# MTG/DeepConvSep

Hardware: NVIDIA H100
Metric: audio_seconds_separated_per_second (higher is better)
Workload: dtype f32

## Files before the change

### deepconvsep_b200/csrc/fft_reg.cuh

```cuda
#pragma once
#include <cuda_runtime.h>
#include "fft.cuh"

namespace dcs {

__device__ __forceinline__ constexpr float cos32(int q) {
  constexpr float t[16] = {1.0f, 0.98078528040323043f, 0.92387953251128674f, 0.83146961230254524f, 0.70710678118654752f,
                           0.55557023301960218f, 0.38268343236508977f, 0.19509032201612825f, 0.0f, -0.19509032201612825f,
                           -0.38268343236508977f, -0.55557023301960218f, -0.70710678118654752f, -0.83146961230254524f,
                           -0.92387953251128674f, -0.98078528040323043f};
  return t[q];
}
__device__ __forceinline__ constexpr float sin32(int q) {
  constexpr float t[16] = {0.0f, 0.19509032201612825f, 0.38268343236508977f, 0.55557023301960218f, 0.70710678118654752f,
                           0.83146961230254524f, 0.92387953251128674f, 0.98078528040323043f, 1.0f, 0.98078528040323043f,
                           0.92387953251128674f, 0.83146961230254524f, 0.70710678118654752f, 0.55557023301960218f,
                           0.38268343236508977f, 0.19509032201612825f};
  return t[q];
}

__host__ __device__ constexpr int brev(int i, int bits) {
  int r = 0;
  for (int k = 0; k < bits; ++k) r |= ((i >> k) & 1) << (bits - 1 - k);
  return r;
}

__device__ __forceinline__ float2 mul_w32(float2 d, int q) {
  if (q == 0) return d;
  if (q == 8) return make_float2(d.y, -d.x);
  if (q == 4) return make_float2(0.70710678118654752f * (d.x + d.y), 0.70710678118654752f * (d.y - d.x));
  if (q == 12) return make_float2(0.70710678118654752f * (d.y - d.x), -0.70710678118654752f * (d.x + d.y));
  const float c = cos32(q), s = sin32(q);
  return make_float2(fmaf(d.x, c, d.y * s), fmaf(d.y, c, -d.x * s));
}

template <int R, int L = R>
__device__ __forceinline__ void fft_dif(float2 (&v)[R]) {
  constexpr int half = L >> 1;
#pragma unroll
  for (int s = 0; s < R; s += L) {
#pragma unroll
    for (int j = 0; j < half; ++j) {
      const float2 a = v[s + j], b = v[s + j + half];
      v[s + j] = cadd(a, b);
      v[s + j + half] = mul_w32(csub(a, b), j * (32 / L));
    }
  }
  if constexpr (L > 2) fft_dif<R, L / 2>(v);
}

template <int T>
struct FftGroup {
  static constexpr int N2 = 32 * T;
  __device__ static __forceinline__ void fill_tw2(float2* tw2, const float2* __restrict__ tw, int tid, int nthreads) {
    for (int i = tid; i < 32 * T; i += nthreads) {
      const int ka = i / T, b = i - ka * T;
      tw2[i] = __ldg(tw + 2 * b * ka);
    }
  }
  static constexpr int PITCH = T + 1;
  static constexpr int SCRATCH = 32 * PITCH;
  static constexpr int Q = 32 / T;
  static constexpr int TBITS = T == 32 ? 5 : 4;

  template <bool TW_SHARED = false>
  __device__ static __forceinline__ void forward(float2 (&v)[32], float2* scr, const float2* __restrict__ tw, int b) {
    fft_dif<32>(v);
#pragma unroll
    for (int ka = 0; ka < 32; ++ka) {
      float2 y = v[brev(ka, 5)];
      if (ka > 0) y = cmul(y, TW_SHARED ? tw[ka * T + b] : __ldg(tw + 2 * b * ka));
      scr[ka * PITCH + b] = y;
    }
    __syncwarp();
    if (T == 32) {
#pragma unroll
      for (int i = 0; i < 32; ++i) v[i] = scr[b * PITCH + i];
      fft_dif<32>(v);
      float2 u[32];
#pragma unroll
      for (int kb = 0; kb < 32; ++kb) u[kb] = v[brev(kb, 5)];
#pragma unroll
      for (int kb = 0; kb < 32; ++kb) v[kb] = u[kb];
    } else {
      float2 u0[16], u1[16];
#pragma unroll
      for (int i = 0; i < 16; ++i) {
        u0[i] = scr[b * PITCH + i];
        u1[i] = scr[(b + 16) * PITCH + i];
      }
      fft_dif<16>(u0);
      fft_dif<16>(u1);
#pragma unroll
      for (int kb = 0; kb < 16; ++kb) {
        v[kb] = u0[brev(kb, 4)];
        v[16 + kb] = u1[brev(kb, 4)];
      }
    }
    __syncwarp();
  }
};

}
```

### deepconvsep_b200/csrc/stft_reg.cu

```cuda
#include "common.cuh"
#include "fft_reg.cuh"
#include "tc.cuh"

namespace dcs {

constexpr int REG_THREADS = 128;
constexpr int ISTFT_THREADS = 256;

template <int T>
__global__ void __launch_bounds__(REG_THREADS)
stft_reg_kernel(const float* __restrict__ audio, int64_t L, int hop, const float* __restrict__ win,
                const float2* __restrict__ tw, float2* __restrict__ X, float* __restrict__ mag,
                float* __restrict__ phase, int64_t ldf, int64_t nframes, float mag_scale, int frames_per_group) {
  using G = FftGroup<T>;
  constexpr int N2 = G::N2, N = 2 * N2, F = N2 + 1, GPC = REG_THREADS / T;
  extern __shared__ __align__(16) float2 scratch[];
  const int tid = threadIdx.x, b = tid % T, gl = tid / T;
  float2* scr = scratch + gl * G::SCRATCH;
  float2* stw = scratch + GPC * G::SCRATCH;
  float2* stw2 = stw + N2;
  float2* swin = stw2 + N2;
  for (int i = tid; i < N2; i += REG_THREADS) stw[i] = __ldg(tw + i);
  G::fill_tw2(stw2, tw, tid, REG_THREADS);
  for (int i = tid; i < N2; i += REG_THREADS) swin[i] = __ldg(reinterpret_cast<const float2*>(win) + i);
  __syncthreads();
  const int64_t g = (int64_t)blockIdx.x * GPC + gl;
  const bool audio_aligned8 = (reinterpret_cast<uintptr_t>(audio) & 7) == 0;
  const int64_t warp_first = ((int64_t)blockIdx.x * GPC + (tid / 32) * (32 / T)) * frames_per_group;
  for (int i = 0; i < frames_per_group; ++i) {
    if (warp_first + i >= nframes) break;
    const int64_t n = g * frames_per_group + i;
    const bool valid = n < nframes;
    const int64_t base = n * hop - N / 2;
    float2 v[32];
    if (valid && base >= 0 && base + N <= L && audio_aligned8) {
      const float2* __restrict__ ap = reinterpret_cast<const float2*>(audio + base);
#pragma unroll
      for (int a = 0; a < 32; ++a) {
        const int idx = a * T + b;
        const float2 w = swin[idx], x = __ldg(ap + idx);
        v[a] = make_float2(x.x * w.x, x.y * w.y);
      }
    } else {
#pragma unroll
      for (int a = 0; a < 32; ++a) {
        const int idx = a * T + b;
        const int64_t s = base + 2 * idx;
        const float2 w = swin[idx];
        const float x0 = (valid && s >= 0 && s < L) ? __ldg(audio + s) : 0.f;
        const float x1 = (valid && s + 1 >= 0 && s + 1 < L) ? __ldg(audio + s + 1) : 0.f;
        v[a] = make_float2(x0 * w.x, x1 * w.y);
      }
    }
    G::template forward<true>(v, scr, stw2, b);
#pragma unroll
    for (int q = 0; q < G::Q; ++q)
#pragma unroll
      for (int kb = 0; kb < T; ++kb) scr[(b + T * q) + 32 * kb] = v[q * T + kb];
    __syncwarp();
    if (valid) {
      const int64_t row = n * ldf;
#pragma unroll 4
      for (int m = 0; m < N2 / T; ++m) {
        const int k = b + T * m;
        const float2 xk = real_post_shared<N2>(scr, stw, k);
        if (X) X[row + k] = xk;
        if (mag) mag[row + k] = mag_scale * sqrtf(xk.x * xk.x + xk.y * xk.y);
        if (phase) phase[row + k] = atan2f(xk.y, xk.x);
      }
      if (b == 0) {
        const float2 z0 = scr[0];
        const float vv = z0.x - z0.y;
        if (X) X[row + N2] = make_float2(vv, 0.f);
        if (mag) mag[row + N2] = mag_scale * fabsf(vv);
        if (phase) phase[row + N2] = atan2f(0.f, vv);
      }
      if (b < ldf - F) {
        if (X) X[row + F + b] = make_float2(0.f, 0.f);
        if (mag) mag[row + F + b] = 0.f;
        if (phase) phase[row + F + b] = 0.f;
      }
    }
    __syncwarp();
  }
}

constexpr int ISTFT_RING = 2;
constexpr size_t SM90_SMEM_OPTIN = 232448;
template <int T>
__host__ __device__ constexpr int istft_rowp() { return (32 * T + 1 + 7) / 8 * 8; }
template <int T>
__host__ __device__ constexpr size_t istft_smem_bytes(int qpc, bool masked) {
  constexpr int GPC = ISTFT_THREADS / T, ROWP = istft_rowp<T>();
  return ((size_t)GPC * FftGroup<T>::SCRATCH + 3 * (size_t)(32 * T) + (size_t)qpc * ISTFT_RING * ROWP) * sizeof(float2) +
         (masked ? (size_t)GPC * ISTFT_RING * ROWP * sizeof(float) : 0) +
         ((size_t)qpc * 2 * ISTFT_RING + (masked ? (size_t)GPC * ISTFT_RING : 0)) * sizeof(uint64_t);
}

template <int T, int HS, bool MASKED>
__device__ __forceinline__ void
istft_reg_body(const float2* __restrict__ S, int64_t nframes, int64_t ldf, int64_t src_stride,
               const float* __restrict__ wsyn, const float* __restrict__ w2, const float2* __restrict__ tw,
               float* __restrict__ out, int64_t Lout, int64_t out_stride, int hops_per_group, int64_t num_hops,
               int64_t groups_per_src, int64_t total_quads, const float* __restrict__ Mk, int64_t m_stride, int nsrc,
               int nx, int qw, int qpc) {
  using G = FftGroup<T>;
  constexpr int N2 = G::N2, N = 2 * N2, hop = 64 * HS, R = N / hop, C0 = (N / 2) / hop, GPC = ISTFT_THREADS / T;
  constexpr int ROWP = istft_rowp<T>();
  constexpr uint32_t XBYTES = (N2 + 2) / 2 * 16;
  constexpr uint32_t MBYTES = (N2 + 4) / 4 * 16;
  extern __shared__ __align__(16) float2 scratch[];
  const int tid = threadIdx.x, b = tid % T, gl = tid / T;
  float2* scr = scratch + gl * G::SCRATCH;
  const int qi = gl / qw, mem = gl - qi * qw;
  const bool in_quad = qi < qpc;
  int64_t gq = (int64_t)blockIdx.x * qpc + (in_quad ? qi : 0);
  bool active = in_quad && gq < total_quads;
  if (gq >= total_quads) gq = total_quads - 1;
  int msrc = 0;
  if constexpr (MASKED) {
    const int nchunk = (nsrc + qw - 1) / qw;
    msrc = (int)(gq % nchunk) * qw + mem;
    gq /= nchunk;
    if (msrc >= nsrc) { active = false; msrc = nsrc - 1; }
  }
  const int src = (int)(gq / groups_per_src);
  const int64_t h0 = (gq % groups_per_src) * hops_per_group;
  const float inv_n2 = 1.0f / (float)N2;
  float2 acc[32];
#pragma unroll
  for (int i = 0; i < 32; ++i) acc[i] = make_float2(0.f, 0.f);
  float* o = out + (int64_t)(MASKED ? msrc * nx + src : src) * out_stride;
  float2 cinv[G::Q * HS];
#pragma unroll
  for (int q = 0; q < G::Q; ++q)
#pragma unroll
    for (int kb = 0; kb < HS; ++kb) {
      const int e = 2 * ((b + T * q) + 32 * kb);
      float c0 = 0.f, c1 = 0.f;
#pragma unroll
      for (int r = 0; r < R; ++r) {
        const float2 ww = __ldg(reinterpret_cast<const float2*>(w2 + e + r * hop));
        c0 += ww.x;
        c1 += ww.y;
      }
      cinv[q * HS + kb] = make_float2(c0 == 0.f ? 1.f : 1.f / c0, c1 == 0.f ? 1.f : 1.f / c1);
    }

  float2* stw = scratch + GPC * G::SCRATCH;
  float2* stw2 = stw + N2;
  float2* swsyn = stw2 + N2;
  float2* xring = swsyn + N2 + (in_quad ? qi : 0) * ISTFT_RING * ROWP;
  float* mring = reinterpret_cast<float*>(swsyn + N2 + qpc * ISTFT_RING * ROWP) + gl * ISTFT_RING * ROWP;
  uint64_t* bars = reinterpret_cast<uint64_t*>(reinterpret_cast<float*>(swsyn + N2 + qpc * ISTFT_RING * ROWP) +
                                               (MASKED ? GPC * ISTFT_RING * ROWP : 0));
  uint64_t* xfull = bars + (in_quad ? qi : 0) * 2 * ISTFT_RING;
  uint64_t* xempty = xfull + ISTFT_RING;
  uint64_t* mfull = bars + qpc * 2 * ISTFT_RING + gl * ISTFT_RING;
  for (int i = tid; i < N2; i += ISTFT_THREADS) stw[i] = __ldg(tw + i);
  G::fill_tw2(stw2, tw, tid, ISTFT_THREADS);
  for (int i = tid; i < N2; i += ISTFT_THREADS) swsyn[i] = __ldg(reinterpret_cast<const float2*>(wsyn) + i);
  if (tid < qpc * ISTFT_RING) {
    tc::mbar_init(bars + (tid / ISTFT_RING) * 2 * ISTFT_RING + tid % ISTFT_RING, 1);
    tc::mbar_init(bars + (tid / ISTFT_RING) * 2 * ISTFT_RING + ISTFT_RING + tid % ISTFT_RING, (uint32_t)qw);
  }
  if (MASKED && tid < GPC * ISTFT_RING) tc::mbar_init(bars + qpc * 2 * ISTFT_RING + tid, 1);
  tc::fence_barrier_init();
  __syncthreads();
  const bool xlane = in_quad && mem == 0 && b == 0;
  const bool glane = in_quad && b == 0;
  const int64_t n_first = h0 + C0 - R + 1, n_last = h0 + hops_per_group - 1 + C0;
  auto fetch_x = [&](int64_t nn) {
    const int k = (int)(nn - n_first), st = k % ISTFT_RING;
    if (k >= ISTFT_RING)
      tc::mbar_wait_relaxed(xempty + st, (uint32_t)((k / ISTFT_RING - 1) & 1));
    if (nn >= 0 && nn < nframes) {
      tc::mbar_arrive_expect_tx(xfull + st, XBYTES);
      tc::bulk_copy_g2s(xring + st * ROWP, S + (int64_t)src * src_stride + nn * ldf, XBYTES, xfull + st);
    } else {
      tc::mbar_arrive(xfull + st);
    }
  };
  auto fetch_m = [&](int64_t nn) {
    const int st = (int)(nn - n_first) % ISTFT_RING;
    if (nn >= 0 && nn < nframes) {
      tc::mbar_arrive_expect_tx(mfull + st, MBYTES);
      tc::bulk_copy_g2s(mring + st * ROWP, Mk + (int64_t)msrc * m_stride + nn * ldf, MBYTES, mfull + st);
    } else {
      tc::mbar_arrive(mfull + st);
    }
  };
  if (xlane) fetch_x(n_first);
  if (MASKED && glane) fetch_m(n_first);
  for (int64_t n = n_first; n <= n_last; ++n) {
    const bool fvalid = in_quad && n >= 0 && n < nframes;
    const int k = (int)(n - n_first), st = k % ISTFT_RING;
    const uint32_t par = (uint32_t)((k / ISTFT_RING) & 1);
    if (n < n_last) {
      if (xlane) fetch_x(n + 1);
      if (MASKED && glane) fetch_m(n + 1);
    }
    const float2* srow = xring + st * ROWP;
    const float* smrow = mring + st * ROWP;
    if (in_quad) {
      tc::mbar_wait(xfull + st, par);
      if constexpr (MASKED) tc::mbar_wait(mfull + st, par);
    }
    float2 v[32];
#pragma unroll
    for (int a = 0; a < 32; ++a) {
      const int idx = a * T + b;
      float2 xk = make_float2(0.f, 0.f), xn = xk;
      if (fvalid) {
        xk = srow[idx];
        xn = srow[N2 - idx];
        if constexpr (MASKED) {
          const float mk = smrow[idx], mn = smrow[N2 - idx];
          xk = make_float2(__fmul_rn(mk, xk.x), __fmul_rn(mk, xk.y));
          xn = make_float2(__fmul_rn(mn, xn.x), __fmul_rn(mn, xn.y));
        }
      }
      if (idx == 0) { xk.y = 0.f; xn.y = 0.f; }
      v[a] = real_pre_conj(xk, xn, stw[idx]);
    }
    __syncwarp();
    if (glane) tc::mbar_arrive(xempty + st);
    G::template forward<true>(v, scr, stw2, b);
#pragma unroll
    for (int q = 0; q < G::Q; ++q)
#pragma unroll
      for (int kb = 0; kb < T; ++kb) {
        const int np = (b + T * q) + 32 * kb;
        const float2 w = swsyn[np];
        const float2 r = v[q * T + kb];
        acc[q * T + kb].x = fmaf(w.x, r.x * inv_n2, acc[q * T + kb].x);
        acc[q * T + kb].y = fmaf(w.y, -r.y * inv_n2, acc[q * T + kb].y);
      }
    const int64_t h = n - C0;
    if (active && h >= h0 && h < num_hops) {
      const bool interior = (n - (R - 1) >= 0) && (n < nframes);
#pragma unroll
      for (int q = 0; q < G::Q; ++q)
#pragma unroll
        for (int kb = 0; kb < HS; ++kb) {
          const int e = 2 * ((b + T * q) + 32 * kb);
          float2 ic = cinv[q * HS + kb];
          if (!interior) {
            float c0 = 0.f, c1 = 0.f;
#pragma unroll
            for (int r = 0; r < R; ++r) {
              const int64_t nf = n - r;
              if (nf >= 0 && nf < nframes) {
                const float2 ww = __ldg(reinterpret_cast<const float2*>(w2 + e + r * hop));
                c0 += ww.x;
                c1 += ww.y;
              }
            }
            ic = make_float2(c0 == 0.f ? 1.f : 1.f / c0, c1 == 0.f ? 1.f : 1.f / c1);
          }
          const int64_t oi = h * hop + e;
          const float2 a2 = acc[q * T + kb];
          if (oi + 1 < Lout) {
            *reinterpret_cast<float2*>(o + oi) = make_float2(a2.x * ic.x, a2.y * ic.y);
          } else if (oi < Lout) {
            o[oi] = a2.x * ic.x;
          }
        }
    }
#pragma unroll
    for (int q = 0; q < G::Q; ++q) {
#pragma unroll
      for (int kb = 0; kb < T - HS; ++kb) acc[q * T + kb] = acc[q * T + kb + HS];
#pragma unroll
      for (int kb = T - HS; kb < T; ++kb) acc[q * T + kb] = make_float2(0.f, 0.f);
    }
  }
}

template <int T, int HS>
__global__ void __launch_bounds__(ISTFT_THREADS, 1)
istft_reg_kernel(const float2* __restrict__ S, int64_t nframes, int64_t ldf, int64_t src_stride,
                 const float* __restrict__ wsyn, const float* __restrict__ w2, const float2* __restrict__ tw,
                 float* __restrict__ out, int64_t Lout, int64_t out_stride, int hops_per_group, int64_t num_hops,
                 int64_t groups_per_src, int64_t total_groups) {
  istft_reg_body<T, HS, false>(S, nframes, ldf, src_stride, wsyn, w2, tw, out, Lout, out_stride, hops_per_group, num_hops,
                               groups_per_src, total_groups, nullptr, 0, 1, 1, 1, ISTFT_THREADS / T);
}

template <int T, int HS>
__global__ void __launch_bounds__(ISTFT_THREADS, 1)
istft_masked_reg_kernel(const float2* __restrict__ X, int64_t nframes, int64_t ldf, int64_t x_plane,
                        const float* __restrict__ Mk, int64_t m_stride, int nsrc, int nx, const float* __restrict__ wsyn,
                        const float* __restrict__ w2, const float2* __restrict__ tw, float* __restrict__ out, int64_t Lout,
                        int64_t out_stride, int hops_per_group, int64_t num_hops, int64_t groups_per_plane,
                        int64_t total_quads, int qw, int qpc) {
  istft_reg_body<T, HS, true>(X, nframes, ldf, x_plane, wsyn, w2, tw, out, Lout, out_stride, hops_per_group, num_hops,
                              groups_per_plane, total_quads, Mk, m_stride, nsrc, nx, qw, qpc);
}

int launch_stft_reg(dcs_stft* p, const float* d_audio, int64_t L, float2* d_X, float* d_mag, float* d_phase,
                    float mag_scale, int64_t ldf, int64_t nframes, cudaStream_t st) {
  const int fpg = 4;
  const float ms = mag_scale / sqrtf((float)p->N);
  if (p->N == 2048) {
    using G = FftGroup<32>;
    const int gpc = REG_THREADS / 32;
    const size_t smem = (gpc * G::SCRATCH + 3 * G::N2) * sizeof(float2);
    DCS_TRY(ensure_smem_attr(stft_reg_kernel<32>, (int)smem));
    const unsigned grid = (unsigned)ceil_div64(nframes, (int64_t)gpc * fpg);
    stft_reg_kernel<32><<<grid, REG_THREADS, smem, st>>>(
        d_audio, L, p->hop, p->d_win, p->d_tw, d_X, d_mag, d_phase, ldf, nframes, ms, fpg);
  } else {
    using G = FftGroup<16>;
    const int gpc = REG_THREADS / 16;
    const size_t smem = (gpc * G::SCRATCH + 3 * G::N2) * sizeof(float2);
    DCS_TRY(ensure_smem_attr(stft_reg_kernel<16>, (int)smem));
    const unsigned grid = (unsigned)ceil_div64(nframes, (int64_t)gpc * fpg);
    stft_reg_kernel<16><<<grid, REG_THREADS, smem, st>>>(
        d_audio, L, p->hop, p->d_win, p->d_tw, d_X, d_mag, d_phase, ldf, nframes, ms, fpg);
  }
  DCS_CHECK_LAUNCH();
  p->ctx->launches++;
  return DCS_OK;
}

bool istft_reg_supported(const dcs_stft* p, const float* d_out, int64_t out_stride) {
  return (p->N == 1024 || p->N == 2048) && (p->hop == 512 || p->hop == 256) && ((uintptr_t)d_out % 8 == 0) &&
         out_stride % 2 == 0;
}

template <int T, int HS>
static int launch_istft_reg_t(dcs_stft* p, const float2* d_S, int nsrc, int64_t nframes, int64_t ldf, int64_t src_stride,
                              float* d_out, int64_t Lout, int64_t out_stride, cudaStream_t st, const float* d_M = nullptr,
                              int64_t m_stride = 0, int nx = 1) {
  constexpr int GPC = ISTFT_THREADS / T;
  const int hop = 64 * HS;
  const int64_t num_hops = ceil_div64(Lout, hop);
  const int64_t target_groups = (int64_t)p->ctx->num_sms * (ISTFT_THREADS / 32) * (32 / T);
  const int nplanes = nsrc * nx;
  int64_t hpg = ceil_div64((int64_t)nplanes * num_hops, target_groups);
  if (hpg < 12) hpg = 12;
  if (hpg > 64) hpg = 64;
  const int64_t groups_per_src = ceil_div64(num_hops, hpg);
  if (d_M) {
    const int qw = nsrc < GPC ? nsrc : GPC;
    int qpc = GPC / qw;
    while (qpc > 1 && istft_smem_bytes<T>(qpc, true) > SM90_SMEM_OPTIN) --qpc;
    const int64_t quads = groups_per_src * nx * ((nsrc + qw - 1) / qw);
    const unsigned grid = (unsigned)ceil_div64(quads, qpc);
    const size_t smem = istft_smem_bytes<T>(qpc, true);
    DCS_TRY(ensure_smem_attr(istft_masked_reg_kernel<T, HS>, (int)smem));
    istft_masked_reg_kernel<T, HS><<<grid, ISTFT_THREADS, smem, st>>>(
        d_S, nframes, ldf, src_stride, d_M, m_stride, nsrc, nx, p->d_wsyn, p->d_w2, p->d_tw, d_out, Lout, out_stride,
        (int)hpg, num_hops, groups_per_src, quads, qw, qpc);
  } else {
    const int64_t total = groups_per_src * nplanes;
    const unsigned grid = (unsigned)ceil_div64(total, GPC);
    const size_t smem = istft_smem_bytes<T>(GPC, false);
    DCS_TRY(ensure_smem_attr(istft_reg_kernel<T, HS>, (int)smem));
    istft_reg_kernel<T, HS><<<grid, ISTFT_THREADS, smem, st>>>(
        d_S, nframes, ldf, src_stride, p->d_wsyn, p->d_w2, p->d_tw, d_out, Lout, out_stride, (int)hpg, num_hops,
        groups_per_src, total);
  }
  DCS_CHECK_LAUNCH();
  p->ctx->launches++;
  return DCS_OK;
}

int launch_istft_reg(dcs_stft* p, const float2* d_S, int nsrc, int64_t nframes, int64_t ldf, int64_t src_stride,
                     float* d_out, int64_t Lout, int64_t out_stride, cudaStream_t st, const float* d_M, int64_t m_stride,
                     int nx) {
#define DCS_ISTFT_REG_CASE(NN, HOP) \
  if (p->N == NN && p->hop == HOP)  \
    return launch_istft_reg_t<NN / 64, HOP / 64>(p, d_S, nsrc, nframes, ldf, src_stride, d_out, Lout, out_stride, st, d_M, m_stride, nx);
  DCS_ISTFT_REG_CASE(2048, 512)
  DCS_ISTFT_REG_CASE(2048, 256)
  DCS_ISTFT_REG_CASE(1024, 512)
  DCS_ISTFT_REG_CASE(1024, 256)
#undef DCS_ISTFT_REG_CASE
  DCS_REQUIRE(false, "istft_reg: unsupported frame size / hop");
}

}
```

Measured before the change: 162,600.

## Restructure ISTFT overlap-add accumulators and halve FFT scratch for masked kernel

The overlap-add accumulator becomes a per-hop ring of P×HV registers, so the per-frame shift loop over all 32 accumulators goes away. Window normalization and the 1/N scale are folded into the shared synthesis window, and the per-thread inverse-coefficient registers are replaced with a shared-memory table. The masked kernel moves to 384 threads with a half-size FFT transpose scratch, done in two passes via forward_split, to fit more warps per block. Per-warp frame offsets and clamp ranges are precomputed into shared memory to simplify the frame loop. This adds complexity and extra syncwarps, and increases register pressure at the higher thread count.

```diff
diff --git a/deepconvsep_b200/csrc/fft_reg.cuh b/deepconvsep_b200/csrc/fft_reg.cuh
--- a/deepconvsep_b200/csrc/fft_reg.cuh
+++ b/deepconvsep_b200/csrc/fft_reg.cuh
@@ -99,6 +99,59 @@
     }
     __syncwarp();
   }
+
+  static constexpr int HALF_SCRATCH = 16 * PITCH;
+  __device__ static __forceinline__ void forward_split(float2 (&v)[32], float2* scr, const float2* tw, int b) {
+    fft_dif<32>(v);
+    auto y = [&](int ka) { return ka > 0 ? cmul(v[brev(ka, 5)], tw[ka * T + b]) : v[0]; };
+    if (T == 32) {
+      const bool hi = (b & 16) != 0;
+      float2 later[16];
+#pragma unroll
+      for (int a = 0; a < 16; ++a) {
+        const float2 lo = y(a), up = y(a + 16);
+        scr[a * PITCH + b] = hi ? up : lo;
+        later[a] = hi ? lo : up;
+      }
+      const float2* row = scr + (b & 15) * PITCH;
+      __syncwarp();
+#pragma unroll
+      for (int i = 0; i < 16; ++i) v[i] = row[(hi ? 16 : 0) + i];
+      __syncwarp();
+#pragma unroll
+      for (int a = 0; a < 16; ++a) scr[a * PITCH + b] = later[a];
+      __syncwarp();
+#pragma unroll
+      for (int i = 0; i < 16; ++i) v[16 + i] = row[(hi ? 0 : 16) + i];
+      fft_dif<32>(v);
+      float2 u[32];
+#pragma unroll
+      for (int kb = 0; kb < 32; ++kb) u[kb] = v[brev(kb, 5)];
+#pragma unroll
+      for (int kb = 0; kb < 32; ++kb) v[kb] = u[kb];
+    } else {
+      float2 u0[16], u1[16];
+#pragma unroll
+      for (int a = 0; a < 16; ++a) scr[a * PITCH + b] = y(a);
+      __syncwarp();
+#pragma unroll
+      for (int i = 0; i < 16; ++i) u0[i] = scr[b * PITCH + i];
+      __syncwarp();
+#pragma unroll
+      for (int a = 0; a < 16; ++a) scr[a * PITCH + b] = y(16 + a);
+      __syncwarp();
+#pragma unroll
+      for (int i = 0; i < 16; ++i) u1[i] = scr[b * PITCH + i];
+      fft_dif<16>(u0);
+      fft_dif<16>(u1);
+#pragma unroll
+      for (int kb = 0; kb < 16; ++kb) {
+        v[kb] = u0[brev(kb, 4)];
+        v[16 + kb] = u1[brev(kb, 4)];
+      }
+    }
+    __syncwarp();
+  }
 };
 
 }
diff --git a/deepconvsep_b200/csrc/stft_reg.cu b/deepconvsep_b200/csrc/stft_reg.cu
--- a/deepconvsep_b200/csrc/stft_reg.cu
+++ b/deepconvsep_b200/csrc/stft_reg.cu
@@ -6,6 +6,8 @@
 
 constexpr int REG_THREADS = 128;
 constexpr int ISTFT_THREADS = 256;
+constexpr int ISTFT_MASKED_THREADS = 384;
+__host__ __device__ constexpr int istft_threads(bool masked) { return masked ? ISTFT_MASKED_THREADS : ISTFT_THREADS; }
 
 template <int T>
 __global__ void __launch_bounds__(REG_THREADS)
@@ -89,12 +91,20 @@
 constexpr size_t SM90_SMEM_OPTIN = 232448;
 template <int T>
 __host__ __device__ constexpr int istft_rowp() { return (32 * T + 1 + 7) / 8 * 8; }
-template <int T>
+template <int T, int HS>
 __host__ __device__ constexpr size_t istft_smem_bytes(int qpc, bool masked) {
-  constexpr int GPC = ISTFT_THREADS / T, ROWP = istft_rowp<T>();
-  return ((size_t)GPC * FftGroup<T>::SCRATCH + 3 * (size_t)(32 * T) + (size_t)qpc * ISTFT_RING * ROWP) * sizeof(float2) +
-         (masked ? (size_t)GPC * ISTFT_RING * ROWP * sizeof(float) : 0) +
-         ((size_t)qpc * 2 * ISTFT_RING + (masked ? (size_t)GPC * ISTFT_RING : 0)) * sizeof(uint64_t);
+  const int gpc = istft_threads(masked) / T, rowp = istft_rowp<T>();
+  const int scr = masked ? FftGroup<T>::HALF_SCRATCH : FftGroup<T>::SCRATCH;
+  return ((size_t)gpc * scr + 3 * (size_t)(32 * T) + 32 * HS + (size_t)qpc * ISTFT_RING * rowp) * sizeof(float2) +
+         (masked ? (size_t)gpc * ISTFT_RING * rowp * sizeof(float) : 0) +
+         ((size_t)qpc * 2 * ISTFT_RING + (masked ? (size_t)gpc * ISTFT_RING : 0) + 6 * (size_t)gpc) * sizeof(uint64_t);
+}
+
+__device__ __forceinline__ float2 real_pre_conj_x2(float2 xk, float2 xn, float2 twk) {
+  const float2 e = make_float2(xk.x + xn.x, xk.y - xn.y);
+  const float2 d = make_float2(xk.x - xn.x, xk.y + xn.y);
+  const float2 o = cmul(d, make_float2(twk.x, -twk.y));
+  return make_float2(e.x - o.y, -(e.y + o.x));
 }
 
 template <int T, int HS, bool MASKED>
@@ -105,13 +115,17 @@
                int64_t groups_per_src, int64_t total_quads, const float* __restrict__ Mk, int64_t m_stride, int nsrc,
                int nx, int qw, int qpc) {
   using G = FftGroup<T>;
-  constexpr int N2 = G::N2, N = 2 * N2, hop = 64 * HS, R = N / hop, C0 = (N / 2) / hop, GPC = ISTFT_THREADS / T;
+  constexpr int N2 = G::N2, N = 2 * N2, hop = 64 * HS, R = N / hop, C0 = (N / 2) / hop;
+  constexpr int THREADS = istft_threads(MASKED), GPC = THREADS / T;
+  constexpr int SCR = MASKED ? G::HALF_SCRATCH : G::SCRATCH;
+  constexpr int P = R - 1;
+  constexpr int HV = G::Q * HS;
   constexpr int ROWP = istft_rowp<T>();
   constexpr uint32_t XBYTES = (N2 + 2) / 2 * 16;
   constexpr uint32_t MBYTES = (N2 + 4) / 4 * 16;
   extern __shared__ __align__(16) float2 scratch[];
   const int tid = threadIdx.x, b = tid % T, gl = tid / T;
-  float2* scr = scratch + gl * G::SCRATCH;
+  float2* scr = scratch + gl * SCR;
   const int qi = gl / qw, mem = gl - qi * qw;
   const bool in_quad = qi < qpc;
   int64_t gq = (int64_t)blockIdx.x * qpc + (in_quad ? qi : 0);
@@ -126,40 +140,45 @@
   }
   const int src = (int)(gq / groups_per_src);
   const int64_t h0 = (gq % groups_per_src) * hops_per_group;
-  const float inv_n2 = 1.0f / (float)N2;
-  float2 acc[32];
-#pragma unroll
-  for (int i = 0; i < 32; ++i) acc[i] = make_float2(0.f, 0.f);
+  float2 acc[P][HV];
+#pragma unroll
+  for (int p = 0; p < P; ++p)
+#pragma unroll
+    for (int i = 0; i < HV; ++i) acc[p][i] = make_float2(0.f, 0.f);
   float* o = out + (int64_t)(MASKED ? msrc * nx + src : src) * out_stride;
-  float2 cinv[G::Q * HS];
-#pragma unroll
-  for (int q = 0; q < G::Q; ++q)
-#pragma unroll
-    for (int kb = 0; kb < HS; ++kb) {
-      const int e = 2 * ((b + T * q) + 32 * kb);
-      float c0 = 0.f, c1 = 0.f;
-#pragma unroll
-      for (int r = 0; r < R; ++r) {
-        const float2 ww = __ldg(reinterpret_cast<const float2*>(w2 + e + r * hop));
-        c0 += ww.x;
-        c1 += ww.y;
-      }
-      cinv[q * HS + kb] = make_float2(c0 == 0.f ? 1.f : 1.f / c0, c1 == 0.f ? 1.f : 1.f / c1);
-    }
-
-  float2* stw = scratch + GPC * G::SCRATCH;
+
+  float2* stw = scratch + GPC * SCR;
   float2* stw2 = stw + N2;
   float2* swsyn = stw2 + N2;
-  float2* xring = swsyn + N2 + (in_quad ? qi : 0) * ISTFT_RING * ROWP;
-  float* mring = reinterpret_cast<float*>(swsyn + N2 + qpc * ISTFT_RING * ROWP) + gl * ISTFT_RING * ROWP;
-  uint64_t* bars = reinterpret_cast<uint64_t*>(reinterpret_cast<float*>(swsyn + N2 + qpc * ISTFT_RING * ROWP) +
+  float2* scinv = swsyn + N2;
+  float2* xring = scinv + 32 * HS + (in_quad ? qi : 0) * ISTFT_RING * ROWP;
+  float* mring = reinterpret_cast<float*>(scinv + 32 * HS + qpc * ISTFT_RING * ROWP) + gl * ISTFT_RING * ROWP;
+  uint64_t* bars = reinterpret_cast<uint64_t*>(reinterpret_cast<float*>(scinv + 32 * HS + qpc * ISTFT_RING * ROWP) +
                                                (MASKED ? GPC * ISTFT_RING * ROWP : 0));
   uint64_t* xfull = bars + (in_quad ? qi : 0) * 2 * ISTFT_RING;
   uint64_t* xempty = xfull + ISTFT_RING;
   uint64_t* mfull = bars + qpc * 2 * ISTFT_RING + gl * ISTFT_RING;
-  for (int i = tid; i < N2; i += ISTFT_THREADS) stw[i] = __ldg(tw + i);
-  G::fill_tw2(stw2, tw, tid, ISTFT_THREADS);
-  for (int i = tid; i < N2; i += ISTFT_THREADS) swsyn[i] = __ldg(reinterpret_cast<const float2*>(wsyn) + i);
+  int64_t* roff = reinterpret_cast<int64_t*>(bars + qpc * 2 * ISTFT_RING + (MASKED ? GPC * ISTFT_RING : 0)) + 6 * gl;
+  int* kr = reinterpret_cast<int*>(roff + 2);
+  for (int i = tid; i < N2; i += THREADS) stw[i] = __ldg(tw + i);
+  G::fill_tw2(stw2, tw, tid, THREADS);
+  const float inv_n = 1.0f / (float)N;
+  for (int i = tid; i < N2; i += THREADS) {
+    const float2 w = __ldg(reinterpret_cast<const float2*>(wsyn) + i);
+    const bool neg = MASKED && T == 32 && (i & 48) == 48;
+    const float sx = w.x * inv_n, sy = -w.y * inv_n;
+    swsyn[i] = neg ? make_float2(-sx, -sy) : make_float2(sx, sy);
+  }
+  for (int i = tid; i < 32 * HS; i += THREADS) {
+    float c0 = 0.f, c1 = 0.f;
+#pragma unroll
+    for (int r = 0; r < R; ++r) {
+      const float2 ww = __ldg(reinterpret_cast<const float2*>(w2 + 2 * i + r * hop));
+      c0 += ww.x;
+      c1 += ww.y;
+    }
+    scinv[i] = make_float2(c0 == 0.f ? 1.f : 1.f / c0, c1 == 0.f ? 1.f : 1.f / c1);
+  }
   if (tid < qpc * ISTFT_RING) {
     tc::mbar_init(bars + (tid / ISTFT_RING) * 2 * ISTFT_RING + tid % ISTFT_RING, 1);
     tc::mbar_init(bars + (tid / ISTFT_RING) * 2 * ISTFT_RING + ISTFT_RING + tid % ISTFT_RING, (uint32_t)qw);
@@ -169,36 +188,54 @@
   __syncthreads();
   const bool xlane = in_quad && mem == 0 && b == 0;
   const bool glane = in_quad && b == 0;
-  const int64_t n_first = h0 + C0 - R + 1, n_last = h0 + hops_per_group - 1 + C0;
-  auto fetch_x = [&](int64_t nn) {
-    const int k = (int)(nn - n_first), st = k % ISTFT_RING;
+  const int64_t n_first = h0 + C0 - R + 1;
+  if (b == 0) {
+    roff[0] = (int64_t)src * src_stride + n_first * ldf;
+    roff[1] = (int64_t)msrc * m_stride + n_first * ldf;
+  }
+  const int nk = hops_per_group + R - 1;
+  auto kclamp = [&](int64_t x) { return (int)(x < 0 ? 0 : x > nk ? nk : x); };
+  if (b == 0) {
+    kr[0] = kclamp(-n_first);
+    kr[1] = kclamp(nframes - n_first);
+    kr[2] = kclamp(R - 1 - n_first);
+    kr[3] = active ? kclamp(num_hops - h0 + R - 1) : 0;
+  }
+  __syncwarp();
+  if (b == 0) {
+    const int64_t lrem = Lout - h0 * hop;
+    roff[4] = reinterpret_cast<int64_t>(o + h0 * hop);
+    roff[5] = lrem > (int64_t)nk * hop ? (int64_t)nk * hop : lrem;
+  }
+  auto fetch_x = [&](int k) {
+    const int st = k % ISTFT_RING, kf0 = kr[0], kf1 = kr[1];
     if (k >= ISTFT_RING)
       tc::mbar_wait_relaxed(xempty + st, (uint32_t)((k / ISTFT_RING - 1) & 1));
-    if (nn >= 0 && nn < nframes) {
+    if (k >= kf0 && k < kf1) {
       tc::mbar_arrive_expect_tx(xfull + st, XBYTES);
-      tc::bulk_copy_g2s(xring + st * ROWP, S + (int64_t)src * src_stride + nn * ldf, XBYTES, xfull + st);
+      tc::bulk_copy_g2s(xring + st * ROWP, S + roff[0] + k * ldf, XBYTES, xfull + st);
     } else {
       tc::mbar_arrive(xfull + st);
     }
   };
-  auto fetch_m = [&](int64_t nn) {
-    const int st = (int)(nn - n_first) % ISTFT_RING;
-    if (nn >= 0 && nn < nframes) {
+  auto fetch_m = [&](int k) {
+    const int st = k % ISTFT_RING, kf0 = kr[0], kf1 = kr[1];
+    if (k >= kf0 && k < kf1) {
       tc::mbar_arrive_expect_tx(mfull + st, MBYTES);
-      tc::bulk_copy_g2s(mring + st * ROWP, Mk + (int64_t)msrc * m_stride + nn * ldf, MBYTES, mfull + st);
+      tc::bulk_copy_g2s(mring + st * ROWP, Mk + roff[1] + k * ldf, MBYTES, mfull + st);
     } else {
       tc::mbar_arrive(mfull + st);
     }
   };
-  if (xlane) fetch_x(n_first);
-  if (MASKED && glane) fetch_m(n_first);
-  for (int64_t n = n_first; n <= n_last; ++n) {
-    const bool fvalid = in_quad && n >= 0 && n < nframes;
-    const int k = (int)(n - n_first), st = k % ISTFT_RING;
+  if (xlane) fetch_x(0);
+  if (MASKED && glane) fetch_m(0);
+  for (int k = 0; k < nk; ++k) {
+    const bool fvalid = in_quad && k >= kr[0] && k < kr[1];
+    const int st = k % ISTFT_RING;
     const uint32_t par = (uint32_t)((k / ISTFT_RING) & 1);
-    if (n < n_last) {
-      if (xlane) fetch_x(n + 1);
-      if (MASKED && glane) fetch_m(n + 1);
+    if (k + 1 < nk) {
+      if (xlane) fetch_x(k + 1);
+      if (MASKED && glane) fetch_m(k + 1);
     }
     const float2* srow = xring + st * ROWP;
     const float* smrow = mring + st * ROWP;
@@ -207,72 +244,92 @@
       if constexpr (MASKED) tc::mbar_wait(mfull + st, par);
     }
     float2 v[32];
-#pragma unroll
-    for (int a = 0; a < 32; ++a) {
-      const int idx = a * T + b;
-      float2 xk = make_float2(0.f, 0.f), xn = xk;
-      if (fvalid) {
-        xk = srow[idx];
-        xn = srow[N2 - idx];
+    if (fvalid) {
+#pragma unroll
+      for (int a = 0; a < 32; ++a) {
+        const int idx = a * T + b;
+        float2 xk = srow[idx], xn = srow[N2 - idx];
         if constexpr (MASKED) {
           const float mk = smrow[idx], mn = smrow[N2 - idx];
           xk = make_float2(__fmul_rn(mk, xk.x), __fmul_rn(mk, xk.y));
           xn = make_float2(__fmul_rn(mn, xn.x), __fmul_rn(mn, xn.y));
         }
-      }
-      if (idx == 0) { xk.y = 0.f; xn.y = 0.f; }
-      v[a] = real_pre_conj(xk, xn, stw[idx]);
+        if (idx == 0) { xk.y = 0.f; xn.y = 0.f; }
+        v[a] = real_pre_conj_x2(xk, xn, stw[idx]);
+      }
+    } else {
+#pragma unroll
+      for (int a = 0; a < 32; ++a) v[a] = make_float2(0.f, 0.f);
     }
     __syncwarp();
     if (glane) tc::mbar_arrive(xempty + st);
-    G::template forward<true>(v, scr, stw2, b);
+    if constexpr (MASKED) G::forward_split(v, scr, stw2, b);
+    else G::template forward<true>(v, scr, stw2, b);
+    float2 fin[HV];
 #pragma unroll
     for (int q = 0; q < G::Q; ++q)
 #pragma unroll
       for (int kb = 0; kb < T; ++kb) {
-        const int np = (b + T * q) + 32 * kb;
-        const float2 w = swsyn[np];
+        const int j = kb / HS, s = q * HS + kb % HS;
+        const float2 w = swsyn[(b + T * q) + 32 * kb];
         const float2 r = v[q * T + kb];
-        acc[q * T + kb].x = fmaf(w.x, r.x * inv_n2, acc[q * T + kb].x);
-        acc[q * T + kb].y = fmaf(w.y, -r.y * inv_n2, acc[q * T + kb].y);
-      }
-    const int64_t h = n - C0;
-    if (active && h >= h0 && h < num_hops) {
-      const bool interior = (n - (R - 1) >= 0) && (n < nframes);
-#pragma unroll
-      for (int q = 0; q < G::Q; ++q)
-#pragma unroll
-        for (int kb = 0; kb < HS; ++kb) {
-          const int e = 2 * ((b + T * q) + 32 * kb);
-          float2 ic = cinv[q * HS + kb];
-          if (!interior) {
+        const float2 prev = j == R - 1 ? make_float2(0.f, 0.f) : acc[j][s];
+        float2& a = j == 0 ? fin[s] : acc[j - 1][s];
+        a = make_float2(fmaf(w.x, r.x, prev.x), fmaf(w.y, r.y, prev.y));
+      }
+    const int4 kq = *reinterpret_cast<const int4*>(kr);
+    const int kf0 = kq.x, kf1 = kq.y, ki0 = kq.z, ks1 = kq.w;
+    if (k >= R - 1 && k < ks1) {
+      const int hk = (k - (R - 1)) * hop;
+      float* const oh0 = reinterpret_cast<float*>(roff[4]);
+      const int lrem = (int)roff[5];
+      auto put = [&](int s, int np, float2 ic) {
+        const int oi = hk + 2 * np;
+        const float2 a2 = fin[s];
+        if (oi + 1 < lrem) {
+          *reinterpret_cast<float2*>(oh0 + oi) = make_float2(a2.x * ic.x, a2.y * ic.y);
+        } else if (oi < lrem) {
+          oh0[oi] = a2.x * ic.x;
+        }
+      };
+      if (k >= ki0 && k < kf1 && hk + hop <= lrem) {
+#pragma unroll
+        for (int q = 0; q < G::Q; ++q)
+#pragma unroll
+          for (int kb = 0; kb < HS; ++kb) {
+            const int np = (b + T * q) + 32 * kb;
+            const float2 a2 = fin[q * HS + kb], ic = scinv[np];
+            *reinterpret_cast<float2*>(oh0 + hk + 2 * np) = make_float2(a2.x * ic.x, a2.y * ic.y);
+          }
+      } else if (k >= ki0 && k < kf1) {
+#pragma unroll
+        for (int q = 0; q < G::Q; ++q)
+#pragma unroll
+          for (int kb = 0; kb < HS; ++kb) {
+            const int np = (b + T * q) + 32 * kb;
+            put(q * HS + kb, np, scinv[np]);
+          }
+      } else {
+#pragma unroll
+        for (int s = 0; s < HV; ++s) scr[s * T + b] = fin[s];
+#pragma unroll
+        for (int q = 0; q < G::Q; ++q)
+#pragma unroll
+          for (int kb = 0; kb < HS; ++kb) {
+            const int np = (b + T * q) + 32 * kb;
             float c0 = 0.f, c1 = 0.f;
 #pragma unroll
             for (int r = 0; r < R; ++r) {
-              const int64_t nf = n - r;
-              if (nf >= 0 && nf < nframes) {
-                const float2 ww = __ldg(reinterpret_cast<const float2*>(w2 + e + r * hop));
+              if (k - r >= kf0 && k - r < kf1) {
+                const float2 ww = __ldg(reinterpret_cast<const float2*>(w2 + 2 * np + r * hop));
                 c0 += ww.x;
                 c1 += ww.y;
               }
             }
-            ic = make_float2(c0 == 0.f ? 1.f : 1.f / c0, c1 == 0.f ? 1.f : 1.f / c1);
+            fin[q * HS + kb] = scr[(q * HS + kb) * T + b];
+            put(q * HS + kb, np, make_float2(c0 == 0.f ? 1.f : 1.f / c0, c1 == 0.f ? 1.f : 1.f / c1));
           }
-          const int64_t oi = h * hop + e;
-          const float2 a2 = acc[q * T + kb];
-          if (oi + 1 < Lout) {
-            *reinterpret_cast<float2*>(o + oi) = make_float2(a2.x * ic.x, a2.y * ic.y);
-          } else if (oi < Lout) {
-            o[oi] = a2.x * ic.x;
-          }
-        }
-    }
-#pragma unroll
-    for (int q = 0; q < G::Q; ++q) {
-#pragma unroll
-      for (int kb = 0; kb < T - HS; ++kb) acc[q * T + kb] = acc[q * T + kb + HS];
-#pragma unroll
-      for (int kb = T - HS; kb < T; ++kb) acc[q * T + kb] = make_float2(0.f, 0.f);
+      }
     }
   }
 }
@@ -288,7 +345,7 @@
 }
 
 template <int T, int HS>
-__global__ void __launch_bounds__(ISTFT_THREADS, 1)
+__global__ void __launch_bounds__(ISTFT_MASKED_THREADS, 1)
 istft_masked_reg_kernel(const float2* __restrict__ X, int64_t nframes, int64_t ldf, int64_t x_plane,
                         const float* __restrict__ Mk, int64_t m_stride, int nsrc, int nx, const float* __restrict__ wsyn,
                         const float* __restrict__ w2, const float2* __restrict__ tw, float* __restrict__ out, int64_t Lout,
@@ -333,32 +390,33 @@
 static int launch_istft_reg_t(dcs_stft* p, const float2* d_S, int nsrc, int64_t nframes, int64_t ldf, int64_t src_stride,
                               float* d_out, int64_t Lout, int64_t out_stride, cudaStream_t st, const float* d_M = nullptr,
                               int64_t m_stride = 0, int nx = 1) {
-  constexpr int GPC = ISTFT_THREADS / T;
+  const bool masked = d_M != nullptr;
+  const int threads = istft_threads(masked), gpc = threads / T;
   const int hop = 64 * HS;
   const int64_t num_hops = ceil_div64(Lout, hop);
-  const int64_t target_groups = (int64_t)p->ctx->num_sms * (ISTFT_THREADS / 32) * (32 / T);
+  const int64_t target_groups = (int64_t)p->ctx->num_sms * gpc;
   const int nplanes = nsrc * nx;
   int64_t hpg = ceil_div64((int64_t)nplanes * num_hops, target_groups);
   if (hpg < 12) hpg = 12;
   if (hpg > 64) hpg = 64;
   const int64_t groups_per_src = ceil_div64(num_hops, hpg);
-  if (d_M) {
-    const int qw = nsrc < GPC ? nsrc : GPC;
-    int qpc = GPC / qw;
-    while (qpc > 1 && istft_smem_bytes<T>(qpc, true) > SM90_SMEM_OPTIN) --qpc;
+  if (masked) {
+    const int qw = nsrc < gpc ? nsrc : gpc;
+    int qpc = gpc / qw;
+    while (qpc > 1 && istft_smem_bytes<T, HS>(qpc, true) > SM90_SMEM_OPTIN) --qpc;
     const int64_t quads = groups_per_src * nx * ((nsrc + qw - 1) / qw);
     const unsigned grid = (unsigned)ceil_div64(quads, qpc);
-    const size_t smem = istft_smem_bytes<T>(qpc, true);
+    const size_t smem = istft_smem_bytes<T, HS>(qpc, true);
     DCS_TRY(ensure_smem_attr(istft_masked_reg_kernel<T, HS>, (int)smem));
-    istft_masked_reg_kernel<T, HS><<<grid, ISTFT_THREADS, smem, st>>>(
+    istft_masked_reg_kernel<T, HS><<<grid, threads, smem, st>>>(
         d_S, nframes, ldf, src_stride, d_M, m_stride, nsrc, nx, p->d_wsyn, p->d_w2, p->d_tw, d_out, Lout, out_stride,
         (int)hpg, num_hops, groups_per_src, quads, qw, qpc);
   } else {
     const int64_t total = groups_per_src * nplanes;
-    const unsigned grid = (unsigned)ceil_div64(total, GPC);
-    const size_t smem = istft_smem_bytes<T>(GPC, false);
+    const unsigned grid = (unsigned)ceil_div64(total, gpc);
+    const size_t smem = istft_smem_bytes<T, HS>(gpc, false);
     DCS_TRY(ensure_smem_attr(istft_reg_kernel<T, HS>, (int)smem));
-    istft_reg_kernel<T, HS><<<grid, ISTFT_THREADS, smem, st>>>(
+    istft_reg_kernel<T, HS><<<grid, threads, smem, st>>>(
         d_S, nframes, ldf, src_stride, p->d_wsyn, p->d_w2, p->d_tw, d_out, Lout, out_stride, (int)hpg, num_hops,
         groups_per_src, total);
   }
```

Measured after the change: 170,400, median of 6. +4.8%, better.
